# thu-wangz17/HermNet

Measured on AMD Instinct MI355X. Metric: atom-steps/sec (energy+forces) on 10k-atom 3-element cell; HBM GB/s vs roofline, higher is better.
Workload: dtype f32; 1 GPU; configs[1]: 10000-atom 3-element fcc alloy (Al/Ni/Cu), HVNet rc=5.0 hidden=128 num_rbf=128 layers=5, E=431340 directed edges, energy+forces per step; config=c2, atoms_total=10000, atoms_owned_rank0=10000, halo_atoms_rank0=0, edges_rank0=431340, tuned_gemm_table=False, gemm_tuning_in_warmup=False, parallelism=1 GPU

## Files before the change

### hermnet_amd/_lib.py

```python
import ctypes
import os

_HERE = os.path.dirname(os.path.abspath(__file__))
LIB_PATH = os.environ.get("HERMNET_LIB_PATH") or os.path.join(_HERE, "csrc", "libhermnet_hip.so")

HN_ENV = {"polynomial": 0, "exponential": 1}
_ERR = {1: "HN_ERR_BAD_ARG (unsupported shape or null pointer)",
        2: "HN_ERR_LDS (weight tile does not fit the 160 KiB LDS)",
        3: "HN_ERR_LAUNCH (kernel launch failed)"}

c_fp = ctypes.c_void_p
ABI_VERSION = 13


class RbfDesc(ctypes.Structure):
    _fields_ = [("offset", c_fp), ("num_rbf", ctypes.c_int), ("inv_rc", ctypes.c_float),
                ("coeff", ctypes.c_float), ("env_kind", ctypes.c_int), ("env_p", ctypes.c_int)]


class Graph(ctypes.Structure):
    _fields_ = [("num_nodes", ctypes.c_int), ("num_edges", ctypes.c_int), ("num_rel", ctypes.c_int),
                ("type_rowptr", c_fp), ("csr_rowptr", c_fp), ("csr_src", c_fp),
                ("csc_rowptr", c_fp), ("csc_tgt", c_fp), ("csc_pos", c_fp),
                ("num_src", ctypes.c_int), ("res_row", c_fp)]


class PendingGrads(ctypes.Structure):
    _fields_ = [(n, c_fp) for n in ("gn_parts", "gvec_parts", "x", "mean", "rstd", "gx1", "gvec1")] + \
               [("num_parts", ctypes.c_int), ("hidden_real", ctypes.c_int)] + \
               [(n, c_fp) for n in ("gxh", "hb", "w2t_frag16", "w1t_frag16")]


class RelationsOut(ctypes.Structure):
    _fields_ = [(n, c_fp) for n in ("node_order", "row_of_node", "z_rows", "row_real", "row_active", "csr_rowptr",
                                    "csr_src", "csr_perm", "src_id", "tgt_id", "shift_csr", "csc_rowptr", "csc_tgt",
                                    "csc_pos", "out_rowptr", "out_edges")]


SIGNATURES = {
    "hermnet_abi_version": (ctypes.c_int, []),
    "hermnet_build_info": (ctypes.c_char_p, []),
    "hermnet_edge_geometry_fwd": (ctypes.c_int, [c_fp, c_fp, c_fp, c_fp, c_fp, c_fp, ctypes.c_int, c_fp, c_fp]),
    "hermnet_edge_geometry_bwd": (ctypes.c_int, [c_fp, c_fp, c_fp, c_fp, c_fp, ctypes.c_int, c_fp, c_fp]),
    "hermnet_edge_geometry_bwd_csc": (ctypes.c_int, [c_fp, c_fp, c_fp, c_fp, ctypes.c_int, ctypes.c_int, c_fp, c_fp]),
    "hermnet_edge_geometry_bwd_virial": (ctypes.c_int, [c_fp, c_fp, c_fp, c_fp, ctypes.c_int, c_fp, c_fp, c_fp, c_fp, c_fp,
                                                        c_fp, c_fp, c_fp, ctypes.c_int, c_fp, c_fp, c_fp]),
    "hermnet_graph_virial_workspace": (ctypes.c_size_t, [ctypes.c_int]),
    "hermnet_graph_virial": (ctypes.c_int, [c_fp, c_fp, c_fp, c_fp, ctypes.c_int, ctypes.c_int, c_fp, ctypes.c_size_t, c_fp, c_fp]),
    "hermnet_message_scatter_fwd": (ctypes.c_int, [ctypes.POINTER(Graph), ctypes.POINTER(RbfDesc), ctypes.c_int,
                                                   c_fp, c_fp, c_fp, c_fp, c_fp, c_fp, c_fp, c_fp, c_fp, c_fp, ctypes.c_int, ctypes.c_int, c_fp]),
    "hermnet_message_scatter_bwd": (ctypes.c_int, [ctypes.POINTER(Graph), ctypes.POINTER(RbfDesc), ctypes.c_int,
                                                   c_fp, c_fp, c_fp, c_fp, c_fp, c_fp, c_fp, c_fp,
                                                   c_fp, c_fp, c_fp, c_fp, ctypes.c_int, c_fp, c_fp,
                                                   c_fp, c_fp, ctypes.c_int, c_fp]),
    "hermnet_edge_radial_table": (ctypes.c_int, [ctypes.POINTER(Graph), ctypes.POINTER(RbfDesc), c_fp, c_fp, c_fp]),
    "hermnet_neighbor_workspace": (ctypes.c_size_t, [ctypes.c_int]),
    "hermnet_neighbor_workspace_for": (ctypes.c_size_t, [ctypes.c_int, ctypes.c_int]),
    "hermnet_neighbor_count": (ctypes.c_int, [c_fp, ctypes.c_int, c_fp, c_fp, c_fp, ctypes.c_double, c_fp,
                                              ctypes.c_size_t, c_fp, c_fp, c_fp]),
    "hermnet_neighbor_count_devcell": (ctypes.c_int, [c_fp, ctypes.c_int, c_fp, ctypes.c_double, c_fp, ctypes.c_size_t,
                                                      c_fp, c_fp, c_fp]),
    "hermnet_neighbor_fill": (ctypes.c_int, [c_fp, ctypes.c_int, c_fp, c_fp, c_fp, ctypes.c_double, c_fp, ctypes.c_size_t,
                                             ctypes.c_long, ctypes.c_float, ctypes.c_int, ctypes.c_int,
                                             c_fp, c_fp, c_fp, c_fp, c_fp]),
    "hermnet_neighbor_fill_padded": (ctypes.c_int, [ctypes.c_int, c_fp, ctypes.c_size_t, ctypes.c_long, ctypes.c_float,
                                                    ctypes.c_int, c_fp, c_fp, c_fp, c_fp]),
    "hermnet_relation_counts": (ctypes.c_int, [c_fp, ctypes.c_int, c_fp, ctypes.c_int, c_fp, c_fp]),
    "hermnet_build_relations_workspace": (ctypes.c_size_t, [ctypes.c_int] * 4),
    "hermnet_build_relations": (ctypes.c_int, [c_fp, c_fp, c_fp, ctypes.c_int, ctypes.c_int, c_fp, ctypes.c_int,
                                               c_fp, ctypes.c_int, c_fp, ctypes.POINTER(RelationsOut), ctypes.c_int, c_fp,
                                               ctypes.c_size_t, c_fp]),
    "hermnet_build_triadic_workspace": (ctypes.c_size_t, [ctypes.c_int] * 4),
    "hermnet_build_triadic": (ctypes.c_int, [c_fp, c_fp, c_fp, ctypes.c_int, ctypes.c_int, c_fp, ctypes.c_int, ctypes.c_int,
                                             c_fp, c_fp, ctypes.POINTER(RelationsOut), c_fp, c_fp, ctypes.c_int, c_fp,
                                             ctypes.c_size_t, c_fp]),
    "hermnet_train_node_op": (ctypes.c_int, [ctypes.c_int, c_fp, ctypes.c_int, c_fp, ctypes.c_int, ctypes.c_long, ctypes.c_int,
                                             ctypes.c_float, ctypes.c_float, c_fp]),
    "hermnet_edge_message_fwd_rows": (ctypes.c_int, [c_fp] * 4 + [ctypes.c_long, ctypes.c_int] + [c_fp] * 5 + [ctypes.c_long] +
                                      [c_fp] * 3),
    "hermnet_edge_message_bwd_rows": (ctypes.c_int, [c_fp] * 6 + [ctypes.c_long, ctypes.c_int] + [c_fp] * 6 + [ctypes.c_long] +
                                      [c_fp] * 5),
    "hermnet_edge_message_bwd2_rows": (ctypes.c_int, [c_fp] * 10 + [ctypes.c_long, ctypes.c_int] + [c_fp] * 6 + [ctypes.c_long] +
                                       [c_fp] * 7),
    "hermnet_segment_sum": (ctypes.c_int, [c_fp, c_fp, c_fp, ctypes.c_long, ctypes.c_int, c_fp, c_fp]),
    "hermnet_edge_message_fwd": (ctypes.c_int, [c_fp] * 4 + [ctypes.c_long, ctypes.c_int] + [c_fp] * 6),
    "hermnet_edge_message_bwd": (ctypes.c_int, [c_fp] * 6 + [ctypes.c_long, ctypes.c_int] + [c_fp] * 9),
    "hermnet_edge_message_bwd2": (ctypes.c_int, [c_fp] * 10 + [ctypes.c_long, ctypes.c_int] + [c_fp] * 11),
    "hermnet_ssilu_fwd": (ctypes.c_int, [c_fp, c_fp, ctypes.c_int, c_fp, ctypes.c_long, ctypes.c_int, c_fp]),
# ... 151 lines not shown
```

### hermnet_amd/csrc/message_bwd_cl.h

```cpp
#pragma once
#include <hip/hip_runtime.h>
#include <stddef.h>

#define HN_EDGE_TABLE_FLOATS 32

struct HnBwdClArgs {
  int N, Nsrc, E, T;
  int identity;
  const int* type_rowptr;
  const int* csc_rowptr;
  const int* csc_tgt;
  const int* csc_pos;
  int R, H;
  const float* table;
  const float4* edge;
  const float* xh;
  const float* xh_bias;
  const float* vec;
  const float* wt;
  const float* brbf;
  const float* gx1;
  const float* gvec1;
  float* gxh;
  float* gvec;
  float* gvec_out;
  float* gx;
  float4* gedge;
  int rows_per_block;
  int xcd_remap;
  const int* src_ranges;
  int num_ranges;
  int win_base, win_rows, win_lo, win_hi, win_accumulate;
};

size_t hn_bwd_cl_lds_bytes(int R);
int hn_bwd_cl_launch(HnBwdClArgs a, bool has_vec, int rows_override, const int* ranges_host, hipStream_t s);
```

### hermnet_amd/csrc/message_bwd_cl.hip

```cpp
#include <hip/hip_runtime.h>
#include <stdint.h>
#include <type_traits>
#include "../../include/hermnet_hip.h"
#include "hermnet_math.h"
#include "message_bwd_cl.h"

namespace {

typedef float hn_f2 __attribute__((ext_vector_type(2)));
typedef unsigned hn_u2 __attribute__((ext_vector_type(2)));
typedef __attribute__((address_space(4))) const float hn_cfloat;
typedef __attribute__((address_space(4))) const int hn_cint;

constexpr int kRec = HN_EDGE_TABLE_FLOATS;

#ifndef HN_NT_TABLE
#define HN_NT_TABLE 1
#endif
__global__ __launch_bounds__(256) void edge_table_kernel(const float4* __restrict__ edge, const int* __restrict__ csc_pos,
                                                         int E, const float* __restrict__ offset, int R, float inv_rc,
                                                         float coeff, int env_kind, int env_p,
                                                         float* __restrict__ table, const int* __restrict__ csc_end) {
  constexpr int kLd = kRec + 4;
  __shared__ __align__(16) float stage[4][64 * kLd];
  const int lane = threadIdx.x & 63, wave = threadIdx.x >> 6;
  const int q0 = (blockIdx.x * 4 + wave) * 64;
  if (q0 >= E) return;
  const int q = q0 + lane;
  const int n_csc = csc_end[0];
  float rec[kRec];
#pragma unroll
  for (int w = 0; w < kRec; ++w) rec[w] = 0.f;
  rec[24] = __int_as_float(HN_PAD);
  rec[25] = __int_as_float(HN_PAD);
  if (q < n_csc) {
    const float4 g = edge[csc_pos[q]];
    const float d_next = edge[csc_pos[min(q + 1, n_csc - 1)]].w;
    const float u = g.w * inv_rc;
    const HnEnv env = hn_envelope(u, env_kind, env_p);
    const int lo = hn_window_lo(u, R);
    const float c0 = inv_rc * env.der, c1 = inv_rc * env.val * 2.0f * coeff;
#pragma unroll
    for (int m = 0; m < HN_TAPS; ++m) {
      int k = lo + m;
      k = k < 0 ? 0 : (k >= R ? R - 1 : k);
      const float diff = u - offset[k];
      const float gm = __expf(coeff * (diff * diff));
      rec[2 * m] = env.val * gm;
      rec[2 * m + 1] = c0 * gm + c1 * (gm * diff);
    }
    rec[24] = __int_as_float(lo + HN_PAD);
    rec[25] = __int_as_float(hn_window_lo(d_next * inv_rc, R) + HN_PAD);
    rec[28] = g.x; rec[29] = g.y; rec[30] = g.z;
    rec[31] = __builtin_amdgcn_rcpf(g.w);
  }
  float* st = stage[wave];
#pragma unroll
  for (int w = 0; w < kRec / 4; ++w)
// ... 506 lines not shown
        rpb += (rpb + 31) / 32;
      }
    }
  }
  a.rows_per_block = rpb;
  long chunks = (a.Nsrc + rpb - 1) / rpb;
  if (a.num_ranges > 0) {
    chunks = 0;
    for (int k = 0; k < a.num_ranges; ++k) {
      const int lo = ranges_host[2 * k], hi = ranges_host[2 * k + 1];
      if (hi > lo) chunks += (hi - lo + rpb - 1) / rpb;
    }
  }
  dim3 grid((unsigned)chunks, (unsigned)ncb, (unsigned)a.T);
  if (!windowed) {
    hipLaunchKernelGGL(k, grid, dim3(1024), lds, s, a);
  } else {
    a.win_base = 0; a.win_rows = split + HN_PAD; a.win_lo = 0; a.win_hi = split; a.win_accumulate = 0;
    hipLaunchKernelGGL(k, grid, dim3(1024), lds, s, a);
    a.win_base = split; a.win_rows = rows_all - split; a.win_lo = split; a.win_hi = 0x7fffffff; a.win_accumulate = 1;
    hipLaunchKernelGGL(k, grid, dim3(1024), lds, s, a);
  }
  if (a.gx == nullptr) return hipGetLastError() == hipSuccess ? HN_OK : HN_ERR_LAUNCH;
  const long n4v = has_vec ? (long)a.Nsrc * 3 * a.H / 4 : 0, n4x = (long)a.Nsrc * a.H / 4;
  const long n4 = n4v > n4x ? n4v : n4x;
  hipLaunchKernelGGL(message_bwd_finish_kernel, dim3((unsigned)((n4 + 255) / 256)), dim3(256), 0, s,
                     has_vec ? reinterpret_cast<const float4*>(a.gvec) : nullptr, a.T, n4v,
                     reinterpret_cast<const float4*>(a.gvec1), reinterpret_cast<const float4*>(a.gx1),
                     a.type_rowptr, a.identity, a.H, reinterpret_cast<float4*>(a.gvec_out),
                     reinterpret_cast<float4*>(a.gx), n4x, a.src_ranges, a.num_ranges);
  return hipGetLastError() == hipSuccess ? HN_OK : HN_ERR_LAUNCH;
}

extern "C" int hermnet_edge_radial_table(const hn_graph* g, const hn_rbf_desc* rbf, const float* edge, float* table,
                                         void* stream) {
  if (!g || !rbf || rbf->num_rbf < 2 || g->num_edges < 0) return HN_ERR_BAD_ARG;
  const int num_edges = g->num_edges;
  if (num_edges == 0) return HN_OK;
  if (!edge || !table || !rbf->offset || !g->csc_pos || !g->csc_rowptr) return HN_ERR_BAD_ARG;
  hipLaunchKernelGGL(edge_table_kernel, dim3((num_edges + 255) / 256), dim3(256), 0, (hipStream_t)stream,
                     reinterpret_cast<const float4*>(edge), g->csc_pos, num_edges, rbf->offset, rbf->num_rbf, rbf->inv_rc,
                     rbf->coeff, rbf->env_kind, rbf->env_p, table,
                     g->csc_rowptr + (size_t)g->num_rel * (size_t)(g->num_src > 0 ? g->num_src : g->num_nodes));
  return hipGetLastError() == hipSuccess ? HN_OK : HN_ERR_LAUNCH;
}
```

### hermnet_amd/csrc/message_kernels.hip

```cpp
#include <hip/hip_runtime.h>
#include <stdint.h>
#include <stdlib.h>
#include "../../include/hermnet_hip.h"
#include "hermnet_math.h"
#include "message_bwd_cl.h"
int hn_option(int option);

#define HN_LDS_ROW (3 * HN_CB)
#ifndef HN_SB
#define HN_SB __builtin_amdgcn_sched_barrier(0)
#endif

namespace {

struct MsgArgs {
  int N, E, T;
  int Nsrc;
  const int* res_row;
  const int* type_rowptr;
  const int* csr_rowptr;
  const int* csr_src;
  const int* csc_rowptr;
  const int* csc_tgt;
  const int* csc_pos;
  const float* offset;
  int R;
  float inv_rc, coeff;
  int env_kind, env_p;
  int H;
  const float* xh;
  const float* vec;
  const float* x;
  const float* wt;
  const float* brbf;
  const float4* edge;
  float* x1;
  float* vec1;
  const float* xh_bias;
  const float* gx1;
  const float* gvec1;
  float* gxh;
  float* gvec;
  float* gx;
  float4* gedge;
  int rows_per_block;
  int xcd_remap;
  const int* row_ranges;
  int zero_unknown;
  int win_base, win_rows, win_lo, win_hi, win_accumulate;
};

constexpr int VW = 4;
constexpr int LPE = 64 / VW;

struct Vec {
  float v[VW];
  __device__ __forceinline__ static Vec zero() {
    Vec r;
#pragma unroll
    for (int i = 0; i < VW; ++i) r.v[i] = 0.f;
    return r;
  }
  __device__ __forceinline__ static Vec load(const float* p) {
    const float4 t = *reinterpret_cast<const float4*>(p);
    Vec r;
    const float* f = reinterpret_cast<const float*>(&t);
#pragma unroll
    for (int i = 0; i < VW; ++i) r.v[i] = f[i];
// ... 118 lines not shown
  for (int m = 0; m < HN_TAPS; m += 2) {
    wb = Vec::load(wcol + (m + 1) * HN_LDS_ROW);
    S0 = v_sfma(g[m], wa, S0);
    if (WITH_DER) S1 = v_sfma(gd[m], wa, S1);
    if (m + 2 < HN_TAPS) wa = Vec::load(wcol + (m + 2) * HN_LDS_ROW);
    S0 = v_sfma(g[m + 1], wb, S0);
    if (WITH_DER) S1 = v_sfma(gd[m + 1], wb, S1);
  }
}

__device__ __forceinline__ int xcd_contiguous(int b, int nb, int on) {
  const int per = nb >> 3;
  if (!on || b >= per * 8) return b;
  return (b & 7) * per + (b >> 3);
}

__device__ __forceinline__ int decode_block(const MsgArgs& a, int bx, int& t, int& r0, int& r1) {
  for (t = 0; t < a.T; ++t) {
    const int lo = a.row_ranges ? a.row_ranges[2 * t] : a.type_rowptr[t];
    const int hi = a.row_ranges ? a.row_ranges[2 * t + 1] : a.type_rowptr[t + 1];
    const int nb = hi > lo ? (hi - lo + a.rows_per_block - 1) / a.rows_per_block : 0;
    if (bx < nb) {
      r0 = lo + bx * a.rows_per_block;
      r1 = min(r0 + a.rows_per_block, hi);
      return -1;
    }
    bx -= nb;
  }
  return bx;
}

struct FwdIn {
  float4 g;
  Vec xs, xa, xb;
  Vec vj[3];
  bool live;
};

template <bool HAS_VEC, int NW, bool WIN>
__global__ __launch_bounds__(NW * 64, NW / 4) void message_scatter_fwd_kernel(MsgArgs a) {
  extern __shared__ __align__(16) float lds[];
  const int tile_rows = WIN ? a.win_rows : a.R + 2 * HN_PAD + 1;
  float* wl = lds;
  float* mu = lds + tile_rows * HN_LDS_ROW;
  float2* tapbase = reinterpret_cast<float2*>(mu + ((a.R + 2 * HN_PAD + 1 + 3) & ~3));

  const int cb = blockIdx.y;
  int t, r0, r1;
  const int surplus = decode_block(a, xcd_contiguous(blockIdx.x, gridDim.x, a.xcd_remap), t, r0, r1);
  if (surplus >= 0) {
    if (surplus == 0 && a.zero_unknown) {
      const int c = cb * HN_CB + (threadIdx.x & 63);
      for (int r = a.type_rowptr[a.T] + (int)(threadIdx.x >> 6); r < a.N; r += NW) {
        a.x1[(size_t)r * a.H + c] = 0.f;
#pragma unroll
        for (int d = 0; d < 3; ++d) a.vec1[((size_t)r * 3 + d) * a.H + c] = 0.f;
      }
    }
    return;
  }
  stage_weights<NW * 64>(a, t, cb, wl, mu, WIN ? a.win_base : 0, tile_rows);
  __syncthreads();

  const int lane = threadIdx.x & 63;
  const int wave = threadIdx.x >> 6;
  const int grp = lane / LPE;
  const int gl = lane % LPE;
  float2* tb = tapbase + (wave * VW + grp) * 16;
  const int H = a.H;
  const int col = cb * HN_CB + VW * gl;
  const float inv_sqrt3h = 0.57735026918962576f * rsqrtf((float)H);
  const float inv_sqrth = rsqrtf((float)H);
  const float* xh_t = a.xh + (size_t)t * a.Nsrc * 3 * H;

  Vec bias[3], xbias[3];
#pragma unroll
  for (int p = 0; p < 3; ++p) {
    bias[p] = Vec::load(a.brbf + (size_t)t * 3 * H + p * H + col);
    xbias[p] = a.xh_bias ? Vec::load(a.xh_bias + (size_t)t * 3 * H + p * H + col) : Vec::zero();
  }
  auto bias_of = [&](int p) { return bias[p]; };
  auto xbias_of = [&](int p) { return xbias[p]; };

  for (int r = r0 + wave; r < r1; r += NW) {
    const int beg = a.csr_rowptr[r], end = a.csr_rowptr[r + 1];
    Vec ax = Vec::zero();
    Vec av[3] = {Vec::zero(), Vec::zero(), Vec::zero()};

    for (int base = beg; base < end; base += 64) {
      const int cnt = min(64, end - base);
      const int my_src = lane < cnt ? a.csr_src[base + lane] : 0;
      const int nit = (cnt + VW - 1) / VW;

      auto load_geom = [&](int it, FwdIn& in) {
        const int idx = VW * it + grp;
        in.live = idx < cnt;
        in.g = a.edge[base + (in.live ? idx : 0)];
      };
      auto load_rows = [&](int it, FwdIn& in) {
        const int j = __shfl(my_src, VW * it + grp, 64);
        const float* xr = xh_t + (size_t)j * 3 * H + col;
        in.xs = Vec::load(xr); in.xa = Vec::load(xr + H); in.xb = Vec::load(xr + 2 * H);
        if (HAS_VEC) {
          const float* vr = a.vec + (size_t)j * 3 * H + col;
#pragma unroll
          for (int d = 0; d < 3; ++d) in.vj[d] = Vec::load(vr + d * H);
        }
      };

      auto load_edges = [&](int it) {
        FwdIn in;
        load_geom(it, in);
        load_rows(it, in);
        return in;
      };

      FwdIn cur = load_edges(0);
      for (int it = 0; it < nit; ++it) {
        FwdIn nxt;
        load_geom(min(it + 1, nit - 1), nxt);
        __builtin_amdgcn_sched_barrier(0);
        const float u = cur.g.w * a.inv_rc;
        const HnEnv env = hn_envelope(u, a.env_kind, a.env_p);
        const int lo = hn_window_lo(u, a.R);
        int trow = lo + HN_PAD;
        bool own = true;
        if (WIN) { own = trow >= a.win_lo && trow < a.win_hi; trow = min(max(trow - a.win_base, 0), a.win_rows - HN_TAPS); }
        const float* wcol = wl + trow * HN_LDS_ROW + VW * gl;
        float g[HN_TAPS], gd[HN_TAPS];
        coop_taps(mu, tb, lo, u, a.coeff, gl);
        rbf_taps<false>(tb, g, gd);
        HN_SB;
        const float lv = (cur.live && own) ? 1.0f : 0.0f;
        const float ev = env.val * lv;
        Vec S0, S1;
        rbf_part<false>(wcol, g, gd, S0, S1);
        ax = v_fma(v_add(cur.xs, xbias_of(0)), v_sfma(ev, S0, v_scale(bias_of(0), lv)), ax);
        HN_SB;
        rbf_part<false>(wcol + 2 * HN_CB, g, gd, S0, S1);
        const Vec mb = v_scale(v_mul(v_add(cur.xb, xbias_of(2)), v_sfma(ev, S0, v_scale(bias_of(2), lv))), inv_sqrth);
        av[0] = v_sfma(cur.g.x, mb, av[0]);
        av[1] = v_sfma(cur.g.y, mb, av[1]);
        av[2] = v_sfma(cur.g.z, mb, av[2]);
        HN_SB;
        if (HAS_VEC) {
          rbf_part<false>(wcol + HN_CB, g, gd, S0, S1);
          const Vec ma = v_scale(v_mul(v_add(cur.xa, xbias_of(1)), v_sfma(ev, S0, v_scale(bias_of(1), lv))), inv_sqrt3h);
#pragma unroll
          for (int d = 0; d < 3; ++d) av[d] = v_fma(cur.vj[d], ma, av[d]);
        }
        HN_SB;
        load_rows(min(it + 1, nit - 1), cur);
        cur.g = nxt.g;
        cur.live = nxt.live;
      }
    }
    const int rres = a.res_row ? a.res_row[r] : r;
    const int c1 = col + grp;
    const size_t xo = (size_t)r * H + c1;
    if (WIN && a.win_accumulate) {
      a.x1[xo] += rows_reduce4(ax) * 0.70710678118654752f;
#pragma unroll
      for (int d = 0; d < 3; ++d) a.vec1[((size_t)r * 3 + d) * H + c1] += rows_reduce4(av[d]);
      continue;
    }
    a.x1[xo] = (a.x[(size_t)rres * H + c1] + rows_reduce4(ax)) * 0.70710678118654752f;
#pragma unroll
    for (int d = 0; d < 3; ++d) {
      const size_t vo = ((size_t)r * 3 + d) * H + c1;
      a.vec1[vo] = (HAS_VEC ? a.vec[((size_t)rres * 3 + d) * H + c1] : 0.f) + rows_reduce4(av[d]);
    }
  }
}

struct BwdIn {
  float4 g;
  Vec gx1;
  Vec gd[3];
  int pos;
  bool live;
};

constexpr int BWD_NW = 8;

template <bool HAS_VEC>
__global__ __launch_bounds__(BWD_NW * 64, BWD_NW / 4) void message_scatter_bwd_kernel(MsgArgs a) {
  constexpr int NW = BWD_NW;
// ... 197 lines not shown
  if (rounds < 1) rounds = 1;
  long wgs = (long)cus * rounds - slack;
  if (wgs < 1) wgs = 1;
  long rpb = (work + wgs - 1) / wgs;
  if (rpb < 8) rpb = 8;
  return (int)rpb;
}

size_t lds_bytes(int R, int tile_rows = 0) {
  const size_t rows = (size_t)(R + 2 * HN_PAD + 1);
  const size_t held = tile_rows > 0 ? (size_t)tile_rows : rows;
  return (held * HN_LDS_ROW + ((rows + 3) & ~(size_t)3)) * sizeof(float) + 16 * 4 * 16 * sizeof(float2) +
         6 * HN_CB * sizeof(float);
}

typedef void (*kern_t)(MsgArgs);

int ensure_lds(kern_t k, size_t lds) {
  constexpr int kMax = 64;
  static kern_t done[kMax];
  static size_t done_lds[kMax];
  static int ndone = 0;
  for (int i = 0; i < ndone; ++i)
    if (done[i] == k && done_lds[i] >= lds) return HN_OK;
  if (hipFuncSetAttribute(reinterpret_cast<const void*>(k), hipFuncAttributeMaxDynamicSharedMemorySize, (int)lds) !=
      hipSuccess)
    return HN_ERR_LDS;
  if (ndone < kMax) { done[ndone] = k; done_lds[ndone] = lds; ++ndone; }
  return HN_OK;
}

}

extern "C" int hermnet_message_scatter_fwd(const hn_graph* g, const hn_rbf_desc* rbf, int hidden,
                                           const float* xh, const float* xh_bias, const float* vec, const float* x,
                                           const float* wt, const float* brbf, const float* edge,
                                           float* x1, float* vec1, const int* target_ranges, int zero_unknown_rows,
                                           int range_rows, void* stream) {
  MsgArgs a = {};
  int rc = fill_args(g, rbf, hidden, a);
  if (rc) return rc;
  if (!xh || !x || !wt || !brbf || !x1 || !vec1 || (g->num_edges > 0 && !edge)) return HN_ERR_BAD_ARG;
  if (a.N == 0) return HN_OK;
  a.xh = xh; a.xh_bias = xh_bias; a.vec = vec; a.x = x; a.wt = wt; a.brbf = brbf;
  a.edge = reinterpret_cast<const float4*>(edge);
  a.x1 = x1; a.vec1 = vec1;
  a.row_ranges = target_ranges; a.zero_unknown = (target_ranges == nullptr) || zero_unknown_rows;
  const int rpb_fwd = hn_option(HN_OPT_FWD_ROWS);
  const int rows = (target_ranges && range_rows > 0 && range_rows < a.N) ? range_rows : a.N;
  a.rows_per_block = pick_rows(rows, hidden / HN_CB, a.T * (hidden / HN_CB), rpb_fwd);
  a.xcd_remap = 1;
  dim3 grid((unsigned)(rows / a.rows_per_block + a.T + 1), (unsigned)(hidden / HN_CB));
  hipStream_t s = reinterpret_cast<hipStream_t>(stream);
  const int nw = vec ? 8 : 16;
  size_t lds = lds_bytes(a.R);
  if (lds > 160 * 1024) {
    const int rows_all = a.R + 2 * HN_PAD + 1, split = (rows_all - HN_PAD + 1) / 2;
    const int held = split + HN_PAD > rows_all - split ? split + HN_PAD : rows_all - split;
    lds = lds_bytes(a.R, held);
    if (lds > 160 * 1024) return HN_ERR_LDS;
    kern_t k = vec ? message_scatter_fwd_kernel<true, 8, true> : message_scatter_fwd_kernel<false, 16, true>;
    if (ensure_lds(k, lds) != HN_OK) return HN_ERR_LDS;
    a.win_base = 0; a.win_rows = split + HN_PAD; a.win_lo = 0; a.win_hi = split; a.win_accumulate = 0;
    hipLaunchKernelGGL(k, grid, dim3(nw * 64), lds, s, a);
    a.win_base = split; a.win_rows = rows_all - split; a.win_lo = split; a.win_hi = 0x7fffffff; a.win_accumulate = 1;
    a.zero_unknown = 0;
    hipLaunchKernelGGL(k, grid, dim3(nw * 64), lds, s, a);
    return hipGetLastError() == hipSuccess ? HN_OK : HN_ERR_LAUNCH;
  }
  kern_t k = vec ? message_scatter_fwd_kernel<true, 8, false> : message_scatter_fwd_kernel<false, 16, false>;
  if (ensure_lds(k, lds) != HN_OK) return HN_ERR_LDS;
  hipLaunchKernelGGL(k, grid, dim3(nw * 64), lds, s, a);
  return hipGetLastError() == hipSuccess ? HN_OK : HN_ERR_LAUNCH;
}

extern "C" int hermnet_message_scatter_bwd(const hn_graph* g, const hn_rbf_desc* rbf, int hidden,
                                           const float* xh, const float* xh_bias, const float* vec,
                                           const float* wt, const float* brbf, const float* edge,
                                           const float* gx1, const float* gvec1,
                                           float* gxh, float* gvec, float* gx, float* gedge,
                                           int split_t, const float* edge_table, float* gvec_partials,
                                           const int* source_ranges, const int* source_ranges_host, int num_ranges,
                                           void* stream) {
  MsgArgs a = {};
  int rc = fill_args(g, rbf, hidden, a);
  if (rc) return rc;
  if (!xh || !wt || !brbf || !gx1 || !gvec1 || !gxh || (g->num_edges > 0 && !gedge)) return HN_ERR_BAD_ARG;
  if (vec && !gvec && gx) return HN_ERR_BAD_ARG;
  const bool no_finish = gx == nullptr;
  if (g->num_edges > 0 && !edge) return HN_ERR_BAD_ARG;
  if (split_t != 0) return HN_ERR_BAD_ARG;
  if (a.N == 0) return HN_OK;
  const int use_cl = hn_option(HN_OPT_BWD_LANES16) == 0;
  const bool virtual_targets = g->num_src > 0 || g->res_row != nullptr;
  const size_t gather_bytes = (size_t)a.N * 3 * hidden * sizeof(float);
  const size_t src_rows = g->num_src > 0 ? (size_t)g->num_src : (size_t)a.N;
  const bool cl_ok = edge_table && gather_bytes < 0xffffffffull &&
                     src_rows * 3 * hidden < 0x7fffffffull &&
                     (!vec || a.T == 1 || gvec_partials);
  if (virtual_targets && !cl_ok) return HN_ERR_BAD_ARG;
  if (num_ranges < 0 || (num_ranges > 0 && !(cl_ok && (use_cl || virtual_targets)))) return HN_ERR_BAD_ARG;
  if (no_finish && !(cl_ok && use_cl && !virtual_targets && (!vec || gvec_partials)))
    return HN_ERR_BAD_ARG;
  if (cl_ok && (use_cl || virtual_targets)) {
    HnBwdClArgs b = {};
    b.N = a.N; b.Nsrc = g->num_src > 0 ? g->num_src : a.N; b.E = a.E; b.T = a.T;
// ... 28 lines not shown
```

### hermnet_amd/hermnet.py

```python
import os
from typing import Dict, List, Union

import torch
from torch import nn

from . import switches
from .elements import atomic_numbers
from .ops import EdgeGeometry, TrueEdgeGradient, edge_radial_table
from .relations import RelationalGraph
from .sharding import HaloExchange, HaloExchangeFeatures, HaloGradReturn, SumAcrossRanks
from .layer import (EdgeFanout, EdgeGradSink, EnergyHead, FusedRelationalLayer, GemmRelationalLayer, LayerWeights, Route,
                    StepState)
from .rmnet import PaiNNModule, RadialBasis, ScaledSiLU, relational_layer


class HeteroVertexConv(nn.Module):

    def __init__(self, mods: Dict[str, nn.Module]):
        super().__init__()
        self.mods = nn.ModuleDict(mods)
        self._weights = None

    def forward(self, data):
        g = data.get("_hn_graph")
        if g is None:
            raise RuntimeError("HeteroVertexConv.forward needs a Data prepared by HVNet.forward")
        halo, data._hn_halo = data.get("_hn_halo"), None
        step = data._hn_step
        li = step.layer
        ready = data.get("_hn_weights")
        w = ready[li] if (ready is not None and ready[li].mods[0] is next(iter(self.mods.values()))) else None
        if w is None and data.get("_hn_edge_embed") is None and switches.fused_layer:
            if self._weights is None:
                self._weights = LayerWeights(self.mods.values())
            w = self._weights.refresh()
        if halo is not None and not (w is not None and w.chain and switches.node_chain
                                     and halo.fwd_early is not None and g.N * 3 * data.x.size(1) * 4 < 2 ** 32
                                     and sum(halo.plan.recv_counts) + sum(halo.plan.send_counts) > 0
                                     and switches.halo_overlap() != "0"):
            data.x, data.vec = HaloExchangeFeatures.apply(data.x, data.vec, halo.plan)
            halo = None
# ... 232 lines not shown
            data._hn_lone = lone
            if lone:
                pass
            elif shard.halo_pos_local:
                pos = HaloGradReturn.apply(pos, shard.atom_plan)
            else:
                pos = HaloExchange.apply(pos, shard.atom_plan)
            if not lone:
                row_plan = shard.row_plan(graph.row_of_node)
        if train and pos.is_cuda:
            from .trainops import embedding_rows
            x = embedding_rows(self.embed.weight, graph.z_rows.long())
        else:
            x = self.embed(graph.z_rows) if train else torch.nn.functional.embedding(graph.z_rows, self.embed.weight.detach())
        H = self.hidden_channels
        Hp = (H + 63) // 64 * 64 if (fused and switches.fused_layer) else H
        if Hp != H:
            x = torch.nn.functional.pad(x, (0, Hp - H))
        data._hn_weights = None
        if fused and switches.fused_layer:
            data._hn_weights = self._refresh_weights(pos.device)
        if train:
            edge, edge_parts = self._edge_geometry_autograd(pos, data.get("cell"), graph)
        else:
            if props is not None and (props.want_virials or props.want_graph_virial):
                edge = EdgeGeometry.apply(pos, data.get("cell"), graph, props)
            else:
                edge = EdgeGeometry.apply(pos, data.get("cell"), graph)

        vec = None
        if not fused and not train:
            edge = TrueEdgeGradient.apply(edge)
        data._hn_graph, data._hn_edge, data._hn_rbf = graph, edge, rbf
        if fused and edge.requires_grad and edge.is_cuda:
            graph.edge_table = edge_radial_table(graph, rbf, edge.detach())
        if fused:
            data._hn_edge_embed = None
        elif train and pos.is_cuda and self.radial_basis.rbf_name == "gaussian" and H % 4 == 0 and graph.T > 0:
            parts = edge_parts
            Ek = graph.rel_edge_total()
            data._hn_edge_embed = self.radial_basis.bucketed(edge[:, 3] if parts is None else parts[1], Ek, graph.T,
                                                             graph.rel_edge_bounds_dev())
            if parts is not None:
                data._hn_edge_embed.set_unit_vectors(edge, parts[0], Ek)
        else:
            data._hn_edge_embed = self.radial_basis(edge[:, 3])
        data.x, data.vec = x, vec
        data._hn_edge_handles = data._hn_halo = data._hn_chain_node = None
        step = data._hn_step = StepState()
        if fused and edge.requires_grad and switches.fused_layer:
            all_known = graph.num_src == 0 and graph.N == graph.type_rowptr_host[-1]
            step.edge_sink = EdgeGradSink(len(self.hermconvs), Hp // 64, graph.E, pos.device, zero=not all_known)
            data._hn_edge_handles = EdgeFanout.apply(edge, step.edge_sink)
        for li, conv in enumerate(self.hermconvs):
            step.layer = li
            data = conv(data)
            if row_plan is not None and li + 1 < len(self.hermconvs):
                data._hn_halo = shard.halo_overlap(graph, nodeops_tile_rows(Hp))
        graph._keep = None
        x = data.x
        if Hp != H:
            x = x[:, :H]

        head_params = (self.out_energy[0].weight, self.out_energy[0].bias, self.out_energy[2].weight,
                       self.out_energy[2].bias)
        single = shard is None and graph.num_graphs == 1
        shard_rows = None
        if (shard is not None and shard.num_graphs == 1 and not train and fused
# ... 139 lines not shown
```

### hermnet_amd/ops.py

```python
import ctypes
from types import SimpleNamespace

import torch

from . import _lib

P = _lib.ptr


class KernelTimer(object):

    def __init__(self, prefix="message_scatter"):
        self.pairs = {}
        self.prefix = (prefix,) if isinstance(prefix, str) else tuple(prefix)

    def launch(self, name, fn):
        if not name.startswith(self.prefix):
            return fn()
        a = torch.cuda.Event(enable_timing=True)
        b = torch.cuda.Event(enable_timing=True)
        a.record()
        rc = fn()
        b.record()
        self.pairs.setdefault(name, []).append((a, b))
# ... 137 lines not shown
            else:
                b = graph.batch32.long()[graph.src_id.long()]
                gcell = torch.zeros(nb, 3, 3, dtype=gD.dtype, device=gD.device).index_add_(0, b, outer)
            gcell = gcell.reshape(ctx.cell_shape)
        return gpos_rows.index_select(0, graph.row_of_node), gcell, None, None


class TrueEdgeGradient(torch.autograd.Function):

    @staticmethod
    def forward(ctx, edge):
        ctx.save_for_backward(edge)
        return edge.clone()

    @staticmethod
    def backward(ctx, g):
        (edge,) = ctx.saved_tensors
        rh, d = edge[:, :3], edge[:, 3:4]
        gr, gd = g[:, :3], g[:, 3:4]
        gD = gd * rh + (gr - (gr * rh).sum(1, keepdim=True) * rh) / d
        return torch.cat([gD, torch.zeros_like(d)], dim=1)


def _msg_fwd(graph, rbf, H, xh, vec, x, w, edge, xh_bias=True, ranges=None, zero_unknown=True, out=None, range_rows=0):
    lib = _lib.load()
    b2 = w.b2 if xh_bias else None
    if out is None:
        x1 = torch.empty(graph.N, H, dtype=x.dtype, device=x.device)
        vec1 = torch.empty(graph.N, 3, H, dtype=x.dtype, device=x.device)
    else:
        x1, vec1 = out
    gs, rs = graph.as_struct(), rbf.struct()
    _lib.check(_launch("message_scatter_fwd" + ("" if vec is not None else "_l0"),
                       lambda: lib.hermnet_message_scatter_fwd(
                           ctypes.byref(gs), ctypes.byref(rs), H, P(xh), P(b2), P(vec), P(x), P(w.wt), P(w.brbf), P(edge),
                           P(x1), P(vec1), P(ranges), 1 if zero_unknown else 0, int(range_rows), _stream())),
               "hermnet_message_scatter_fwd")
    return x1, vec1


def _msg_bwd(graph, rbf, H, xh, vec, w, edge, gx1, gvec1, gedge, xh_bias=True, ranges=None, out=None, finish=True):
    lib = _lib.load()
    b2 = w.b2 if xh_bias else None
    if not finish:
        if out is None:
            gxh = torch.empty_like(xh)
            part = None if vec is None else torch.empty((graph.T,) + tuple(vec.shape), dtype=vec.dtype, device=vec.device)
        else:
            gxh, part = out
        rd, rh, nr = None, None, 0
        if ranges is not None:
            rd, host = ranges
            nr = len(host)
            rh = (ctypes.c_int * (2 * nr))(*[v for lo_hi in host for v in lo_hi])
        gs, rs = graph.as_struct(), rbf.struct()
        _lib.check(_launch("message_scatter_bwd" + ("" if vec is not None else "_l0"),
                           lambda: lib.hermnet_message_scatter_bwd(
                               ctypes.byref(gs), ctypes.byref(rs), H, P(xh), P(b2), P(vec), P(w.wt), P(w.brbf), P(edge),
                               P(gx1), P(gvec1), P(gxh), None, None, P(gedge), 0, P(graph.edge_table), P(part),
                               P(rd), rh, nr, _stream())),
                   "hermnet_message_scatter_bwd")
        return gxh, part
    if out is None:
        gxh = torch.empty_like(xh)
        gvec = None if vec is None else torch.empty_like(vec)
        gx = torch.empty(xh.size(1), H, dtype=gx1.dtype, device=gx1.device)
        part = None
        if graph.edge_table is not None and vec is not None and graph.T > 1:
            part = torch.empty((graph.T,) + tuple(vec.shape), dtype=vec.dtype, device=vec.device)
    else:
# ... 16 lines not shown


class MessageScatter(torch.autograd.Function):

    @staticmethod
    def forward(ctx, xh, vec, x, edge, wt, brbf, graph, rbf):
        _require_gpu(x, "MessageScatter")
        H = x.size(1)
        xh = xh.contiguous()
        vec_c = None if vec is None else vec.contiguous()
        w = SimpleNamespace(wt=wt, brbf=brbf)
        x1, vec1 = _msg_fwd(graph, rbf, H, xh, vec_c, x.contiguous(), w, edge, xh_bias=False)
        ctx.save_for_backward(xh, vec_c, edge, wt, brbf)
        ctx.graph, ctx.rbf, ctx.H = graph, rbf, H
        return x1, vec1

    @staticmethod
    def backward(ctx, gx1, gvec1):
        xh, vec, edge, wt, brbf = ctx.saved_tensors
        graph, rbf, H = ctx.graph, ctx.rbf, ctx.H
        gedge = torch.zeros(H // 64, graph.E, 4, dtype=torch.float32, device=gx1.device)
        gxh, gvec, gx = _msg_bwd(graph, rbf, H, xh, vec, SimpleNamespace(wt=wt, brbf=brbf), edge, gx1.contiguous(),
                                 gvec1.contiguous(), gedge, xh_bias=False)
        return gxh, gvec, gx, gedge.sum(0), None, None, None, None


def edge_radial_table(graph, rbf, edge):
    E = edge.size(0)
    table = torch.empty(E + 1, 32, dtype=torch.float32, device=edge.device)
    gs, rs = graph.as_struct(), rbf.struct()
    _lib.check(_launch("edge_radial_table", lambda: _lib.load().hermnet_edge_radial_table(
        ctypes.byref(gs), ctypes.byref(rs), _lib.ptr(edge), _lib.ptr(table), _stream())), "hermnet_edge_radial_table")
    return table
```

### hermnet_amd/relations.py

```python
import os

import torch

from . import switches

_COUNT_CACHE = []
_CONST_CACHE = {}


def _cached_i32(values, dev):
    key = ("i32", values, str(dev))
    t = _CONST_CACHE.get(key)
    if t is None:
        if len(_CONST_CACHE) > 64:
            _CONST_CACHE.clear()
        t = _CONST_CACHE[key] = torch.tensor(list(values), dtype=torch.int32, device=dev)
    return t


def _cached_u8(values, dev):
    key = ("u8", values, str(dev))
    t = _CONST_CACHE.get(key)
    if t is None:
        t = _CONST_CACHE[key] = torch.tensor(list(values), dtype=torch.uint8, device=dev)
    return t


class RelationalGraph(object):

    __slots__ = ("N", "E", "T", "num_atoms", "uniform", "block", "node_order", "row_of_node", "z_rows",
                 "type_rowptr", "type_rowptr_host", "csr_rowptr", "csr_src", "csr_perm", "csc_rowptr", "csc_tgt",
                 "csc_pos", "out_rowptr", "out_edges", "src_id", "tgt_id", "shift", "row_active", "row_real",
                 "batch_rows", "batch32", "num_graphs", "graph_perm", "graph_lengths", "device", "_cstruct", "_rel_bounds",
                 "edge_table", "num_src", "res_row", "triadic_pairs", "src_real", "_rowptr_c", "src_ranges", "_row_keys",
                 "_upd_tile", "ready", "_keep", "_edge_atoms64", "_edge_sum_keys", "_row_graph", "_all_known")

    def __init__(self):
        self._cstruct = None
        self._rel_bounds = None
        self._all_known = False
        self._rowptr_c = None
        self._upd_tile = None
        self._row_keys = None
        self.edge_table = None
        self.num_src = 0
        self.res_row = None
        self.triadic_pairs = 0
        self.src_real = None
        self.src_ranges = None
        self._edge_atoms64 = None
        self._edge_sum_keys = None
        self._row_graph = None
        self._keep = None

    def rel_edge_bounds(self):
        if self._rel_bounds is None:
            self._rel_bounds = self.csr_rowptr[self.type_rowptr.long()].tolist()
        return self._rel_bounds

    def rel_edge_total(self):
        if self._all_known:
            return self.E
        return self.rel_edge_bounds()[self.T]

    def rel_edge_bounds_dev(self):
        return self.csr_rowptr[self.type_rowptr.long()]

    @staticmethod
    def build(atomic_number, edge_index, z_list, edge_shift=None, batch=None, rel_active=None, uniform=None):
        if atomic_number.is_cuda and switches.native_relations:
            return RelationalGraph._build_native(atomic_number, edge_index, z_list, edge_shift, batch, rel_active, uniform)
        return RelationalGraph._build_torch(atomic_number, edge_index, z_list, edge_shift, batch, rel_active, uniform)

    @staticmethod
    def _layout(cnt_host, T, uniform):
        known = sum(cnt_host[:T])
        block = max(cnt_host[:T]) if T > 0 else 0
# ... 388 lines not shown
```

### include/hermnet_hip.h

```cpp
#ifndef HERMNET_HIP_H
#define HERMNET_HIP_H

#include <stddef.h>

#ifdef __cplusplus
extern "C" {
#endif

#define HN_OK 0
#define HN_ERR_BAD_ARG 1
#define HN_ERR_LDS 2
#define HN_ERR_LAUNCH 3

#define HN_ENV_POLYNOMIAL 0
#define HN_ENV_EXPONENTIAL 1

int hermnet_abi_version(void);
const char* hermnet_build_info(void);

#define HN_OPT_FWD_ROWS 4
#define HN_OPT_BWD_ROWS 5
#define HN_OPT_BWD_CL_ROWS 6
#define HN_OPT_BWD_LANES16 7
#define HN_OPT_NODE_CHAIN_WIDE 8
// ... 83 lines not shown
int hermnet_edge_geometry_fwd(const float* pos, const int* src_id, const int* tgt_id,
                              const float* shift, const float* cell, const int* batch,
                              int num_edges, float* edge , void* stream);

int hermnet_edge_geometry_bwd(const float* gD, const int* in_rowptr, const int* in_edges,
                              const int* out_rowptr, const int* out_edges,
                              int num_nodes, float* gpos, void* stream);
int hermnet_edge_geometry_bwd_csc(const float* gD, const int* csr_rowptr, const int* csc_rowptr, const int* csc_pos,
                                  int num_rel, int num_nodes, float* gpos, void* stream);
int hermnet_edge_geometry_bwd_virial(const float* gD, const int* csr_rowptr, const int* csc_rowptr, const int* csc_pos,
                                     int num_rel, const int* out_rowptr, const int* out_edges, const float* pos,
                                     const int* src_id, const int* tgt_id, const float* shift, const float* cell,
                                     const int* batch, int num_nodes, float* gpos, float* atom_virial, void* stream);
size_t hermnet_graph_virial_workspace(int num_nodes);
int hermnet_graph_virial(const float* atom_virial, const long* row_of_node, const long* graph_perm, const int* batch,
                         int num_nodes, int num_graphs, void* workspace, size_t workspace_bytes, float* graph_virial,
                         void* stream);

int hermnet_message_scatter_fwd(const hn_graph* g, const hn_rbf_desc* rbf, int hidden,
                                const float* xh, const float* xh_bias, const float* vec, const float* x,
                                const float* wt, const float* brbf, const float* edge,
                                float* x1, float* vec1, const int* target_ranges, int zero_unknown_rows, int range_rows,
                                void* stream);

int hermnet_message_scatter_bwd(const hn_graph* g, const hn_rbf_desc* rbf, int hidden,
                                const float* xh, const float* xh_bias, const float* vec,
                                const float* wt, const float* brbf, const float* edge,
                                const float* gx1, const float* gvec1,
                                float* gxh, float* gvec, float* gx, float* gedge, int split_t,
                                const float* edge_table, float* gvec_partials,
                                const int* source_ranges, const int* source_ranges_host, int num_ranges, void* stream);

int hermnet_edge_radial_table(const hn_graph* g, const hn_rbf_desc* rbf, const float* edge, float* table, void* stream);

int hermnet_ssilu_fwd(const float* h, const float* bias, int rows_per_bias, float* a, long rows, int cols,
                      void* stream);
int hermnet_ssilu_bwd(const float* g, const float* h, const float* bias, int rows_per_bias, float* gh,
                      int N, int T, int C, long g_stride_n, long g_stride_t, void* stream);
int hermnet_layernorm_fwd(const float* x, float* n, float* mean, float* rstd, int rows, int hidden, int hidden_real,
                          float eps, void* stream);
int hermnet_layernorm_bwd(const float* g, const float* x, const float* mean, const float* rstd, const float* add,
                          float* gx, int rows, int hidden, int hidden_real, void* stream);
int hermnet_update_mid(const float* vp, const float* x1, float* vdot, float* xin, int rows, int hidden,
                       void* stream);
int hermnet_update_out(const float* q, const float* qbias , int rows_per_bias,
                       const float* vdot, const float* vp, const float* x1,
                       const float* vec1, const float* row_mask, float* x_out, float* vec_out,
                       int num_nodes, int num_known, int hidden, void* stream);
int hermnet_update_out_bwd(const float* gx_out, const float* gvec_out, const float* q,
                           const float* qbias, int rows_per_bias, const float* vdot,
                           const float* vp, const float* row_mask, float* gq, float* gvdot, float* gvp,
                           float* gx1, float* gvec1, int num_nodes, int num_known, int hidden, void* stream);
int hermnet_update_mid_bwd(const float* gvdot, const float* gxin, const float* vp, const float* xin,
                           float* gvp, float* gx1, int rows, int hidden, void* stream);

int hermnet_energy_head_fwd(const float* h, const float* w, const float* b, const float* row_mask, float* e,
                            int rows, int cols, void* stream);
int hermnet_energy_head_bwd(const float* ge, const float* h, const float* w, const float* row_mask, float* gh,
                            int rows, int cols, void* stream);

int hermnet_energy_head_fused_fwd(const float* x, const float* w0t, const float* b0, const float* w2, const float* b2,
                                  const float* row_mask, float* h, float* e, int rows, int hidden, int cols,
                                  void* stream);
int hermnet_energy_head_fused_bwd(const float* ge, const float* h, const float* w0, const float* w2,
                                  const float* row_mask, float* gx, int rows, int hidden, int cols, void* stream);

// ... 141 lines not shown
```

Before: 3.668 million atom-steps/s.

## Precompute per-edge forward RBF taps once and reuse across message layers

Extends the edge table kernel with extra blocks that compute, per edge in CSR order, the 12 gaussian taps, the envelope value and the window row, and write them to a 16-float record. The forward message-scatter kernel gets a REC template variant that loads one float per lane from this record instead of recomputing envelope, window and exp taps cooperatively. That removes repeated transcendental work across the 5 layers, at the cost of an extra E×16 float buffer (HBM reads per edge per layer) and a larger launch grid for the table kernel.

```diff
diff --git a/hermnet_amd/_lib.py b/hermnet_amd/_lib.py
--- a/hermnet_amd/_lib.py
+++ b/hermnet_amd/_lib.py
@@ -54,6 +54,10 @@
                                                    c_fp, c_fp, c_fp, c_fp, ctypes.c_int, c_fp, c_fp,
                                                    c_fp, c_fp, ctypes.c_int, c_fp]),
     "hermnet_edge_radial_table": (ctypes.c_int, [ctypes.POINTER(Graph), ctypes.POINTER(RbfDesc), c_fp, c_fp, c_fp]),
+    "hermnet_edge_radial_tables": (ctypes.c_int, [ctypes.POINTER(Graph), ctypes.POINTER(RbfDesc), c_fp, c_fp, c_fp, c_fp]),
+    "hermnet_message_scatter_fwd_taps": (ctypes.c_int, [ctypes.POINTER(Graph), ctypes.POINTER(RbfDesc), ctypes.c_int,
+                                                        c_fp, c_fp, c_fp, c_fp, c_fp, c_fp, c_fp, c_fp, c_fp, c_fp, c_fp,
+                                                        ctypes.c_int, ctypes.c_int, c_fp]),
     "hermnet_neighbor_workspace": (ctypes.c_size_t, [ctypes.c_int]),
     "hermnet_neighbor_workspace_for": (ctypes.c_size_t, [ctypes.c_int, ctypes.c_int]),
     "hermnet_neighbor_count": (ctypes.c_int, [c_fp, ctypes.c_int, c_fp, c_fp, c_fp, ctypes.c_double, c_fp,
diff --git a/hermnet_amd/csrc/message_bwd_cl.h b/hermnet_amd/csrc/message_bwd_cl.h
--- a/hermnet_amd/csrc/message_bwd_cl.h
+++ b/hermnet_amd/csrc/message_bwd_cl.h
@@ -3,6 +3,7 @@
 #include <stddef.h>
 
 #define HN_EDGE_TABLE_FLOATS 32
+#define HN_FWD_TAPS_FLOATS 16
 
 struct HnBwdClArgs {
   int N, Nsrc, E, T;
diff --git a/hermnet_amd/csrc/message_bwd_cl.hip b/hermnet_amd/csrc/message_bwd_cl.hip
--- a/hermnet_amd/csrc/message_bwd_cl.hip
+++ b/hermnet_amd/csrc/message_bwd_cl.hip
@@ -17,13 +17,55 @@
 #ifndef HN_NT_TABLE
 #define HN_NT_TABLE 1
 #endif
+__device__ __forceinline__ float fwd_envelope_val(float u, int kind, int p) {
+#pragma clang fp contract(off)
+  if (kind != 0 || !(u < 1.0f)) return hn_envelope(u, kind, p).val;
+  const float up = hn_powi(u, p - 1) * u;
+  const float w = 1.0f - u;
+  const float fp = (float)p;
+  const float inner = __builtin_fmaf(0.5f * fp * (fp + 1.0f), w, fp);
+  const float q = 1.0f + w * inner;
+  return __builtin_fmaf(-q, up, 1.0f);
+}
 __global__ __launch_bounds__(256) void edge_table_kernel(const float4* __restrict__ edge, const int* __restrict__ csc_pos,
                                                          int E, const float* __restrict__ offset, int R, float inv_rc,
                                                          float coeff, int env_kind, int env_p,
-                                                         float* __restrict__ table, const int* __restrict__ csc_end) {
+                                                         float* __restrict__ table, const int* __restrict__ csc_end,
+                                                         float* __restrict__ fwd_taps, int csc_blocks) {
   constexpr int kLd = kRec + 4;
   __shared__ __align__(16) float stage[4][64 * kLd];
   const int lane = threadIdx.x & 63, wave = threadIdx.x >> 6;
+  if ((int)blockIdx.x >= csc_blocks) {
+    constexpr int kF = HN_FWD_TAPS_FLOATS, kLdF = kF + 4;
+    const int e0 = (((int)blockIdx.x - csc_blocks) * 4 + wave) * 64;
+    if (e0 >= E) return;
+    const float u = edge[min(e0 + lane, E - 1)].w * inv_rc;
+    const float env_val = fwd_envelope_val(u, env_kind, env_p);
+    const int lo = hn_window_lo(u, R);
+    float t[kF];
+#pragma unroll
+    for (int m = 0; m < HN_TAPS; ++m) {
+      int k = lo + m;
+      k = k < 0 ? 0 : (k >= R ? R - 1 : k);
+      const float diff = u - offset[k];
+      t[m] = __expf(coeff * (diff * diff));
+    }
+    t[12] = env_val;
+    t[13] = __int_as_float(lo + HN_PAD);
+    t[14] = t[15] = 0.f;
+    float* st = stage[wave];
+#pragma unroll
+    for (int w = 0; w < kF / 4; ++w)
+      *reinterpret_cast<float4*>(st + lane * kLdF + 4 * w) = make_float4(t[4 * w], t[4 * w + 1], t[4 * w + 2], t[4 * w + 3]);
+    const int nrec = min(64, E - e0);
+    float4* out = reinterpret_cast<float4*>(fwd_taps + (size_t)e0 * kF);
+#pragma unroll
+    for (int j = 0; j < kF / 4; ++j) {
+      const int idx = j * 64 + lane, r = idx / (kF / 4), w = idx % (kF / 4);
+      if (r < nrec) out[idx] = *reinterpret_cast<const float4*>(st + r * kLdF + 4 * w);
+    }
+    return;
+  }
   const int q0 = (blockIdx.x * 4 + wave) * 64;
   if (q0 >= E) return;
   const int q = q0 + lane;
@@ -596,15 +638,22 @@
   return hipGetLastError() == hipSuccess ? HN_OK : HN_ERR_LAUNCH;
 }
 
-extern "C" int hermnet_edge_radial_table(const hn_graph* g, const hn_rbf_desc* rbf, const float* edge, float* table,
-                                         void* stream) {
+extern "C" int hermnet_edge_radial_tables(const hn_graph* g, const hn_rbf_desc* rbf, const float* edge, float* table,
+                                          float* fwd_taps, void* stream) {
   if (!g || !rbf || rbf->num_rbf < 2 || g->num_edges < 0) return HN_ERR_BAD_ARG;
   const int num_edges = g->num_edges;
   if (num_edges == 0) return HN_OK;
   if (!edge || !table || !rbf->offset || !g->csc_pos || !g->csc_rowptr) return HN_ERR_BAD_ARG;
-  hipLaunchKernelGGL(edge_table_kernel, dim3((num_edges + 255) / 256), dim3(256), 0, (hipStream_t)stream,
+  const int csc_blocks = (num_edges + 255) / 256;
+  hipLaunchKernelGGL(edge_table_kernel, dim3(fwd_taps ? 2 * csc_blocks : csc_blocks), dim3(256), 0, (hipStream_t)stream,
                      reinterpret_cast<const float4*>(edge), g->csc_pos, num_edges, rbf->offset, rbf->num_rbf, rbf->inv_rc,
                      rbf->coeff, rbf->env_kind, rbf->env_p, table,
-                     g->csc_rowptr + (size_t)g->num_rel * (size_t)(g->num_src > 0 ? g->num_src : g->num_nodes));
+                     g->csc_rowptr + (size_t)g->num_rel * (size_t)(g->num_src > 0 ? g->num_src : g->num_nodes), fwd_taps,
+                     csc_blocks);
   return hipGetLastError() == hipSuccess ? HN_OK : HN_ERR_LAUNCH;
 }
+
+extern "C" int hermnet_edge_radial_table(const hn_graph* g, const hn_rbf_desc* rbf, const float* edge, float* table,
+                                         void* stream) {
+  return hermnet_edge_radial_tables(g, rbf, edge, table, nullptr, stream);
+}
diff --git a/hermnet_amd/csrc/message_kernels.hip b/hermnet_amd/csrc/message_kernels.hip
--- a/hermnet_amd/csrc/message_kernels.hip
+++ b/hermnet_amd/csrc/message_kernels.hip
@@ -34,6 +34,7 @@
   const float* wt;
   const float* brbf;
   const float4* edge;
+  const float* fwd_taps;
   float* x1;
   float* vec1;
   const float* xh_bias;
@@ -218,12 +219,13 @@
 
 struct FwdIn {
   float4 g;
+  float rec;
   Vec xs, xa, xb;
   Vec vj[3];
   bool live;
 };
 
-template <bool HAS_VEC, int NW, bool WIN>
+template <bool HAS_VEC, int NW, bool WIN, bool REC>
 __global__ __launch_bounds__(NW * 64, NW / 4) void message_scatter_fwd_kernel(MsgArgs a) {
   extern __shared__ __align__(16) float lds[];
   const int tile_rows = WIN ? a.win_rows : a.R + 2 * HN_PAD + 1;
@@ -282,6 +284,9 @@
         const int idx = VW * it + grp;
         in.live = idx < cnt;
         in.g = a.edge[base + (in.live ? idx : 0)];
+        if (REC) {
+          in.rec = a.fwd_taps[(size_t)(base + (in.live ? idx : 0)) * HN_FWD_TAPS_FLOATS + gl];
+        }
       };
       auto load_rows = [&](int it, FwdIn& in) {
         const int j = __shfl(my_src, VW * it + grp, 64);
@@ -306,19 +311,35 @@
         FwdIn nxt;
         load_geom(min(it + 1, nit - 1), nxt);
         __builtin_amdgcn_sched_barrier(0);
-        const float u = cur.g.w * a.inv_rc;
-        const HnEnv env = hn_envelope(u, a.env_kind, a.env_p);
-        const int lo = hn_window_lo(u, a.R);
-        int trow = lo + HN_PAD;
+        float g[HN_TAPS], gd[HN_TAPS];
+        float env_val;
+        int trow;
+        if (REC) {
+          float t[HN_FWD_TAPS_FLOATS];
+          float* tf = reinterpret_cast<float*>(tb);
+          tf[gl] = cur.rec;
+#pragma unroll
+          for (int q = 0; q < 3; ++q) *reinterpret_cast<float4*>(t + 4 * q) = *reinterpret_cast<const float4*>(tf + 4 * q);
+          *reinterpret_cast<float2*>(t + 12) = *reinterpret_cast<const float2*>(tf + 12);
+#pragma unroll
+          for (int m = 0; m < HN_TAPS; ++m) g[m] = t[m];
+          env_val = t[12];
+          trow = __float_as_int(t[13]);
+        } else {
+          const float u = cur.g.w * a.inv_rc;
+          const HnEnv env = hn_envelope(u, a.env_kind, a.env_p);
+          const int lo = hn_window_lo(u, a.R);
+          env_val = env.val;
+          trow = lo + HN_PAD;
+          coop_taps(mu, tb, lo, u, a.coeff, gl);
+          rbf_taps<false>(tb, g, gd);
+        }
         bool own = true;
         if (WIN) { own = trow >= a.win_lo && trow < a.win_hi; trow = min(max(trow - a.win_base, 0), a.win_rows - HN_TAPS); }
         const float* wcol = wl + trow * HN_LDS_ROW + VW * gl;
-        float g[HN_TAPS], gd[HN_TAPS];
-        coop_taps(mu, tb, lo, u, a.coeff, gl);
-        rbf_taps<false>(tb, g, gd);
         HN_SB;
         const float lv = (cur.live && own) ? 1.0f : 0.0f;
-        const float ev = env.val * lv;
+        const float ev = env_val * lv;
         Vec S0, S1;
         rbf_part<false>(wcol, g, gd, S0, S1);
         ax = v_fma(v_add(cur.xs, xbias_of(0)), v_sfma(ev, S0, v_scale(bias_of(0), lv)), ax);
@@ -339,6 +360,7 @@
         load_rows(min(it + 1, nit - 1), cur);
         cur.g = nxt.g;
         cur.live = nxt.live;
+        if (REC) cur.rec = nxt.rec;
       }
     }
     const int rres = a.res_row ? a.res_row[r] : r;
@@ -602,11 +624,11 @@
 
 }
 
-extern "C" int hermnet_message_scatter_fwd(const hn_graph* g, const hn_rbf_desc* rbf, int hidden,
-                                           const float* xh, const float* xh_bias, const float* vec, const float* x,
-                                           const float* wt, const float* brbf, const float* edge,
-                                           float* x1, float* vec1, const int* target_ranges, int zero_unknown_rows,
-                                           int range_rows, void* stream) {
+extern "C" int hermnet_message_scatter_fwd_taps(const hn_graph* g, const hn_rbf_desc* rbf, int hidden,
+                                                const float* xh, const float* xh_bias, const float* vec, const float* x,
+                                                const float* wt, const float* brbf, const float* edge,
+                                                const float* fwd_taps, float* x1, float* vec1, const int* target_ranges,
+                                                int zero_unknown_rows, int range_rows, void* stream) {
   MsgArgs a = {};
   int rc = fill_args(g, rbf, hidden, a);
   if (rc) return rc;
@@ -614,6 +636,7 @@
   if (a.N == 0) return HN_OK;
   a.xh = xh; a.xh_bias = xh_bias; a.vec = vec; a.x = x; a.wt = wt; a.brbf = brbf;
   a.edge = reinterpret_cast<const float4*>(edge);
+  a.fwd_taps = fwd_taps;
   a.x1 = x1; a.vec1 = vec1;
   a.row_ranges = target_ranges; a.zero_unknown = (target_ranges == nullptr) || zero_unknown_rows;
   const int rpb_fwd = hn_option(HN_OPT_FWD_ROWS);
@@ -629,7 +652,8 @@
     const int held = split + HN_PAD > rows_all - split ? split + HN_PAD : rows_all - split;
     lds = lds_bytes(a.R, held);
     if (lds > 160 * 1024) return HN_ERR_LDS;
-    kern_t k = vec ? message_scatter_fwd_kernel<true, 8, true> : message_scatter_fwd_kernel<false, 16, true>;
+    kern_t k = fwd_taps ? (vec ? message_scatter_fwd_kernel<true, 8, true, true> : message_scatter_fwd_kernel<false, 16, true, true>)
+                        : (vec ? message_scatter_fwd_kernel<true, 8, true, false> : message_scatter_fwd_kernel<false, 16, true, false>);
     if (ensure_lds(k, lds) != HN_OK) return HN_ERR_LDS;
     a.win_base = 0; a.win_rows = split + HN_PAD; a.win_lo = 0; a.win_hi = split; a.win_accumulate = 0;
     hipLaunchKernelGGL(k, grid, dim3(nw * 64), lds, s, a);
@@ -638,10 +662,20 @@
     hipLaunchKernelGGL(k, grid, dim3(nw * 64), lds, s, a);
     return hipGetLastError() == hipSuccess ? HN_OK : HN_ERR_LAUNCH;
   }
-  kern_t k = vec ? message_scatter_fwd_kernel<true, 8, false> : message_scatter_fwd_kernel<false, 16, false>;
+  kern_t k = fwd_taps ? (vec ? message_scatter_fwd_kernel<true, 8, false, true> : message_scatter_fwd_kernel<false, 16, false, true>)
+                      : (vec ? message_scatter_fwd_kernel<true, 8, false, false> : message_scatter_fwd_kernel<false, 16, false, false>);
   if (ensure_lds(k, lds) != HN_OK) return HN_ERR_LDS;
   hipLaunchKernelGGL(k, grid, dim3(nw * 64), lds, s, a);
   return hipGetLastError() == hipSuccess ? HN_OK : HN_ERR_LAUNCH;
+}
+
+extern "C" int hermnet_message_scatter_fwd(const hn_graph* g, const hn_rbf_desc* rbf, int hidden,
+                                           const float* xh, const float* xh_bias, const float* vec, const float* x,
+                                           const float* wt, const float* brbf, const float* edge,
+                                           float* x1, float* vec1, const int* target_ranges, int zero_unknown_rows,
+                                           int range_rows, void* stream) {
+  return hermnet_message_scatter_fwd_taps(g, rbf, hidden, xh, xh_bias, vec, x, wt, brbf, edge, nullptr, x1, vec1,
+                                          target_ranges, zero_unknown_rows, range_rows, stream);
 }
 
 extern "C" int hermnet_message_scatter_bwd(const hn_graph* g, const hn_rbf_desc* rbf, int hidden,
diff --git a/hermnet_amd/hermnet.py b/hermnet_amd/hermnet.py
--- a/hermnet_amd/hermnet.py
+++ b/hermnet_amd/hermnet.py
@@ -6,7 +6,7 @@
 
 from . import switches
 from .elements import atomic_numbers
-from .ops import EdgeGeometry, TrueEdgeGradient, edge_radial_table
+from .ops import EdgeGeometry, TrueEdgeGradient, edge_radial_tables
 from .relations import RelationalGraph
 from .sharding import HaloExchange, HaloExchangeFeatures, HaloGradReturn, SumAcrossRanks
 from .layer import (EdgeFanout, EdgeGradSink, EnergyHead, FusedRelationalLayer, GemmRelationalLayer, LayerWeights, Route,
@@ -305,8 +305,9 @@
         if not fused and not train:
             edge = TrueEdgeGradient.apply(edge)
         data._hn_graph, data._hn_edge, data._hn_rbf = graph, edge, rbf
+        graph.fwd_taps = None
         if fused and edge.requires_grad and edge.is_cuda:
-            graph.edge_table = edge_radial_table(graph, rbf, edge.detach())
+            graph.edge_table, graph.fwd_taps = edge_radial_tables(graph, rbf, edge.detach())
         if fused:
             data._hn_edge_embed = None
         elif train and pos.is_cuda and self.radial_basis.rbf_name == "gaussian" and H % 4 == 0 and graph.T > 0:
diff --git a/hermnet_amd/ops.py b/hermnet_amd/ops.py
--- a/hermnet_amd/ops.py
+++ b/hermnet_amd/ops.py
@@ -193,10 +193,10 @@
         x1, vec1 = out
     gs, rs = graph.as_struct(), rbf.struct()
     _lib.check(_launch("message_scatter_fwd" + ("" if vec is not None else "_l0"),
-                       lambda: lib.hermnet_message_scatter_fwd(
+                       lambda: lib.hermnet_message_scatter_fwd_taps(
                            ctypes.byref(gs), ctypes.byref(rs), H, P(xh), P(b2), P(vec), P(x), P(w.wt), P(w.brbf), P(edge),
-                           P(x1), P(vec1), P(ranges), 1 if zero_unknown else 0, int(range_rows), _stream())),
-               "hermnet_message_scatter_fwd")
+                           P(graph.fwd_taps), P(x1), P(vec1), P(ranges), 1 if zero_unknown else 0, int(range_rows), _stream())),
+               "hermnet_message_scatter_fwd_taps")
     return x1, vec1
 
 
@@ -279,3 +279,14 @@
     _lib.check(_launch("edge_radial_table", lambda: _lib.load().hermnet_edge_radial_table(
         ctypes.byref(gs), ctypes.byref(rs), _lib.ptr(edge), _lib.ptr(table), _stream())), "hermnet_edge_radial_table")
     return table
+
+
+def edge_radial_tables(graph, rbf, edge):
+    E = edge.size(0)
+    table = torch.empty(E + 1, 32, dtype=torch.float32, device=edge.device)
+    taps = torch.empty(E, 16, dtype=torch.float32, device=edge.device)
+    gs, rs = graph.as_struct(), rbf.struct()
+    _lib.check(_launch("edge_radial_table", lambda: _lib.load().hermnet_edge_radial_tables(
+        ctypes.byref(gs), ctypes.byref(rs), _lib.ptr(edge), _lib.ptr(table), _lib.ptr(taps), _stream())),
+        "hermnet_edge_radial_tables")
+    return table, taps
diff --git a/hermnet_amd/relations.py b/hermnet_amd/relations.py
--- a/hermnet_amd/relations.py
+++ b/hermnet_amd/relations.py
@@ -32,7 +32,7 @@
                  "type_rowptr", "type_rowptr_host", "csr_rowptr", "csr_src", "csr_perm", "csc_rowptr", "csc_tgt",
                  "csc_pos", "out_rowptr", "out_edges", "src_id", "tgt_id", "shift", "row_active", "row_real",
                  "batch_rows", "batch32", "num_graphs", "graph_perm", "graph_lengths", "device", "_cstruct", "_rel_bounds",
-                 "edge_table", "num_src", "res_row", "triadic_pairs", "src_real", "_rowptr_c", "src_ranges", "_row_keys",
+                 "edge_table", "fwd_taps", "num_src", "res_row", "triadic_pairs", "src_real", "_rowptr_c", "src_ranges", "_row_keys",
                  "_upd_tile", "ready", "_keep", "_edge_atoms64", "_edge_sum_keys", "_row_graph", "_all_known")
 
     def __init__(self):
@@ -43,6 +43,7 @@
         self._upd_tile = None
         self._row_keys = None
         self.edge_table = None
+        self.fwd_taps = None
         self.num_src = 0
         self.res_row = None
         self.triadic_pairs = 0
diff --git a/include/hermnet_hip.h b/include/hermnet_hip.h
--- a/include/hermnet_hip.h
+++ b/include/hermnet_hip.h
@@ -139,6 +139,13 @@
                                 const int* source_ranges, const int* source_ranges_host, int num_ranges, void* stream);
 
 int hermnet_edge_radial_table(const hn_graph* g, const hn_rbf_desc* rbf, const float* edge, float* table, void* stream);
+int hermnet_edge_radial_tables(const hn_graph* g, const hn_rbf_desc* rbf, const float* edge, float* table, float* fwd_taps,
+                               void* stream);
+int hermnet_message_scatter_fwd_taps(const hn_graph* g, const hn_rbf_desc* rbf, int hidden,
+                                     const float* xh, const float* xh_bias, const float* vec, const float* x,
+                                     const float* wt, const float* brbf, const float* edge, const float* fwd_taps,
+                                     float* x1, float* vec1, const int* target_ranges, int zero_unknown_rows,
+                                     int range_rows, void* stream);
 
 int hermnet_ssilu_fwd(const float* h, const float* bias, int rows_per_bias, float* a, long rows, int cols,
                       void* stream);
```

After: 3.707 million atom-steps/s, median of 6. 1.01x the previous value.
